# maelaubert/VulkanSift

Hardware: AMD Instinct MI355X
Metric: SIFT detect+match frames/sec (640x480, ~2k kp) (higher is better)
Workload: dtype f32

## Files before the change

vulkansift_amd/csrc/hip/features.hip:

```cpp
#include <hip/hip_runtime.h>
#include <stdint.h>
#include <stdlib.h>
#include <type_traits>

#include "../detmath.h"
#include "features_math.h"
#include "multi.h"
#include "records.h"
#include "vksift_hip.h"
#include "wave.h"

namespace
{

struct FeatArgs
{
  const float *gauss;
  uint32_t fp16;
  int w, h, pitch;
  uint64_t plane_stride, img_stride;
  uint8_t *feats;
  uint64_t feat_img_stride;
  uint32_t cap;
  uint32_t *found;
  uint32_t found_img_stride;
  float *ori_ang;
  uint32_t *ori_cnt;
  uint64_t ori_img_stride;
  uint32_t max_keep;
  uint32_t use_vlfeat;
  const float *desc_fp_tab;
  uint32_t desc_fp_tab_len;
  uint32_t sec;
};

struct ImageView
{
  uint32_t found, n;
  uint8_t *feats;
  int w, h, pitch;
  size_t plane;
};
__device__ __forceinline__ ImageView image_view(const FeatArgs &a, int b)
{
  ImageView v;
  v.found = a.found[(size_t)b * a.found_img_stride];
  v.n = v.found < a.cap ? v.found : a.cap;
  v.feats = a.feats + (size_t)b * a.feat_img_stride;
  v.w = a.w, v.h = a.h, v.pitch = a.pitch;
  v.plane = (size_t)a.plane_stride;
  return v;
}

struct KeyHead
{
  const float *rec;
  float scale_x, scale_y, sigma, theta;
  int octave_idx;
  __amdgpu_buffer_rsrc_t rs;
};
template <bool F16>
__device__ __forceinline__ KeyHead keypoint_head(const FeatArgs &a, const ImageView &v, int b, uint32_t k)
{
  KeyHead kh;
  kh.rec = (const float *)(v.feats + (size_t)k * VKSIFT_RECORD_BYTES);
  const uint32_t scale_idx = (uint32_t)__builtin_amdgcn_readfirstlane((int)((const uint32_t *)kh.rec)[4]);
  kh.octave_idx = ((const int *)kh.rec)[5];
  kh.sigma = kh.rec[6];
  kh.scale_x = kh.rec[2], kh.scale_y = kh.rec[3], kh.theta = kh.rec[7];
  kh.rs = layer_rsrc(a.gauss, (size_t)b * a.img_stride + (size_t)scale_idx * v.plane, v.pitch, v.h, F16);
  return kh;
}

template <bool IMG_FAST, bool F16>
__global__ void __launch_bounds__(256) k_orientation(Multi<FeatArgs> m)
{
  const VBlock vb = vblock(m);
  const FeatArgs &a = m.oct[vb.o];
  __shared__ uint32_t s_hist[4][36];
  const int lane = threadIdx.x & 63, wave = threadIdx.x >> 6;
  const int b = (int)(IMG_FAST ? vb.x : vb.y);
  const ImageView g = image_view(a, b);
  uint32_t *hist = s_hist[wave];

  const uint32_t bk = IMG_FAST ? vb.y : vb.x, nbk = IMG_FAST ? vb.gy : vb.gx;
  for (uint32_t k = bk * 4 + wave; k < g.n; k += nbk * 4)
  {
    if (lane < 36)
      hist[lane] = 0;
    __builtin_amdgcn_wave_barrier();
    float fp = 0.f;
    {
      const KeyHead kh = keypoint_head<F16>(a, g, b, k);
      float lambda = 1.5f * (kh.sigma * dm_pow2i(-kh.octave_idx));
      int r = (int)floorf(3 * lambda);
      float es = -1.f / (2.f * lambda * lambda);
      const bool may_clamp = (2.f * (float)(r + 1) * (float)(r + 1)) * es < -87.f;

      float gsum = 1.f;
      for (int cb = 0; cb <= r; cb += 64)
      {
        int i = cb + lane;
        float e = (i >= 1 && i <= r) ? dm_expf(es * (float)(i * i)) : 0.f;
        int lim = r - cb < 63 ? r - cb : 63;
        for (int j = 0; j <= lim; j++)
        {
          float ej = __shfl(e, j, 64);
          if (cb + j >= 1)
            gsum += 2.f * ej;
        }
      }
      float M = (gsum * gsum) * sqrtf(2.f);
      fp = (float)(1u << (uint32_t)(30 - dm_ceil_log2f(M)));

      float rsx = roundf(kh.scale_x), rsy = roundf(kh.scale_y);
      int box = 2 * r + 1;
      int npix = box * box;
      const float rbox = __builtin_amdgcn_rcpf((float)box);
      const bool small_box = box < 32768;
      const int step_q = small_box ? (int)(64.5f * rbox) : 64 / box, step_r = 64 - step_q * box;
      int py = small_box ? (int)(((float)lane + 0.5f) * rbox) : lane / box, px = lane - py * box;
      auto accumulate = [&](float sdx2, float tr, float tl, float td, float tu) {
        const float gradX = 0.5f * (tr - tl);
        const float gradY = 0.5f * (td - tu);
        const float xe = sdx2 * es;
        float e = dm_expf_core_nonpos(fmaxf(xe, -87.3f));
        if (may_clamp)
          e = xe < -87.3f ? 0.f : e;
        float ori, len;
        bool odd;
        grad_polar<true>(gradX, gradY, &ori, &len, &odd);
        float x36 = wrap_2pi(ori) * 36.f;
        float fbin = angle_bin<true>(x36);
        odd |= angle_bin_odd(x36);
        if (__builtin_expect(__ballot(odd) != 0ull, 0))
        {
          grad_polar<false>(gradX, gradY, &ori, &len, nullptr);
          fbin = angle_bin<false>(wrap_2pi(ori) * 36.f);
        }
        const float mag = e * len;
        int bin = (int)fbin;
        bin = bin >= 36 ? bin - 36 : bin;
        atomicAdd(&hist[bin], (uint32_t)(mag * fp));
      };
      const int cxi = (int)rsx, cyi = (int)rsy;
      const int pitch4 = g.pitch * 4;
      auto window = [&](auto INTERIOR) {
        for (int pix = lane; pix < npix; pix += 64)
        {
          const int dy = py - r, dx = px - r;
          px += step_r, py += step_q;
          if (px >= box)
            px -= box, py++;
          const float sdx = (rsx + (float)dx) - kh.scale_x;
          const float sdy = (rsy + (float)dy) - kh.scale_y;
          const float d2 = (sdx * sdx) + (sdy * sdy);
          if constexpr (decltype(INTERIOR)::value)
          {
            const unsigned v0 = (__umul24((unsigned)(cyi + dy - 1), (unsigned)g.pitch) + (unsigned)(cxi + dx - 1)) * 4u;
            accumulate(d2, tap_ld<F16>(kh.rs, v0 + 8u, pitch4), tap_ld<F16>(kh.rs, v0, pitch4), tap_ld<F16>(kh.rs, v0 + 4u, 2 * pitch4), tap_ld<F16>(kh.rs, v0 + 4u, 0));
          }
          else
          {
            const int gx = cxi + dx, gy = cyi + dy;
            if ((gx < 1 || gx >= (g.w - 1) || gy < 1 || gy >= (g.h - 1)) && (d2 > (float)(r * r)))
              continue;
            const bool xin = (unsigned)gx < (unsigned)g.w, yin = (unsigned)gy < (unsigned)g.h;
            const unsigned o0 = (__umul24((unsigned)gy, (unsigned)g.pitch) + (unsigned)gx) * 4u;
            const unsigned o_r = (yin && (unsigned)(gx + 1) < (unsigned)g.w) ? o0 + 4u : 0x80000000u;
            const unsigned o_l = (yin && (unsigned)(gx - 1) < (unsigned)g.w) ? o0 - 4u : 0x80000000u;
            const unsigned o_d = (xin && (unsigned)(gy + 1) < (unsigned)g.h) ? (__umul24((unsigned)(gy + 1), (unsigned)g.pitch) + (unsigned)gx) * 4u : 0x80000000u;
            const unsigned o_u = (xin && (unsigned)(gy - 1) < (unsigned)g.h) ? (__umul24((unsigned)(gy - 1), (unsigned)g.pitch) + (unsigned)gx) * 4u : 0x80000000u;
            accumulate(d2, tap_ld<F16>(kh.rs, o_r, 0), tap_ld<F16>(kh.rs, o_l, 0), tap_ld<F16>(kh.rs, o_d, 0), tap_ld<F16>(kh.rs, o_u, 0));
          }
        }
      };
      if (cxi - r >= 1 && cxi + r <= g.w - 2 && cyi - r >= 1 && cyi + r <= g.h - 2)
        window(std::true_type{});
      else
        window(std::false_type{});
    }
    __builtin_amdgcn_wave_barrier();
    {
      const int li = lane < 36 ? lane : 0;
      uint32_t hv = hist[li];
      const int lm = (li + 35) % 36, lp = (li + 1) % 36;
#pragma unroll
      for (int it = 0; it < 6; it++)
      {
        uint32_t hm = __shfl(hv, lm, 64), hp = __shfl(hv, lp, 64);
        hv = (uint32_t)dm_div_3((float)(hm + hv + hp));
      }
      uint32_t hm = __shfl(hv, lm, 64), hp = __shfl(hv, lp, 64);
      const uint32_t mx = wave_max_u32(lane < 36 ? hv : 0u);
      bool peak = lane < 36 && ((float)hv >= (0.8f * (float)mx)) && (hv > hm) && (hv > hp);
      unsigned long long pm = __ballot(peak);
      uint32_t npk = (uint32_t)__popcll(pm);
      if (peak)
      {
        uint32_t rank = ballot_rank(pm, lane);
        if (rank < a.max_keep)
        {
          uint32_t num = hm - hp;
          uint32_t den = hm - (2u * hv) + hp;
          float idx = (float)lane + 0.5f * ((float)num / (float)den);
          float ang = (idx + 0.5f) * (2.f * PI_F) / 36.f;
          a.ori_ang[((size_t)b * a.ori_img_stride + k) * VKSIFT_HIP_MAX_ORI + rank] = ang;
        }
      }
      if (lane == 0)
        a.ori_cnt[(size_t)b * a.ori_img_stride + k] = npk < a.max_keep ? npk : a.max_keep;
    }
    __builtin_amdgcn_wave_barrier();
  }
}

__global__ void __launch_bounds__(1024) k_orientation_finalize(Multi<FeatArgs> m)
{
  __shared__ uint32_t wave_tot[16];
  __shared__ uint32_t carry_s;
  const VBlock vb = vblock(m);
  const FeatArgs &a = m.oct[vb.o];
  const int b = (int)vb.x;
  const int lane = threadIdx.x & 63, wave = threadIdx.x >> 6;
  const ImageView g = image_view(a, b);
  const uint32_t *cnt = a.ori_cnt + (size_t)b * a.ori_img_stride;
  const float *ang = a.ori_ang + (size_t)b * a.ori_img_stride * VKSIFT_HIP_MAX_ORI;
  if (threadIdx.x == 0)
    carry_s = 0;
  __syncthreads();
  for (uint32_t base = 0; base < g.n; base += 1024)
  {
    uint32_t k = base + threadIdx.x;
    uint32_t c = k < g.n ? cnt[k] : 0u;
    uint32_t v = c > 1 ? c - 1 : 0u;
    const uint32_t incl = wave_scan_incl_u32(v, lane);
    if (lane == 63)
      wave_tot[wave] = incl;
    __syncthreads();
    uint32_t wave_base = 0;
    for (int wv = 0; wv < wave; wv++)
      wave_base += wave_tot[wv];
    uint32_t carry = carry_s;
    uint32_t excl = carry + wave_base + incl - v;
    if (k < g.n && c >= 1)
    {
      uint32_t *rec = (uint32_t *)(g.feats + (size_t)k * VKSIFT_RECORD_BYTES);
      rec[7] = __float_as_uint(ang[(size_t)k * VKSIFT_HIP_MAX_ORI]);
      for (uint32_t j = 1; j < c; j++)
      {
        uint32_t idx = g.found + excl + (j - 1);
        if (idx < a.cap)
        {
          uint32_t *dst = (uint32_t *)(g.feats + (size_t)idx * VKSIFT_RECORD_BYTES);
#pragma unroll
          for (int q = 0; q < (int)VKSIFT_RECORD_HEAD_WORDS; q++)
            dst[q] = rec[q];
          dst[7] = __float_as_uint(ang[(size_t)k * VKSIFT_HIP_MAX_ORI + j]);
        }
      }
    }
    __syncthreads();
    if (threadIdx.x == 1023)
      carry_s = carry + wave_base + incl;
    __syncthreads();
  }
  if (threadIdx.x == 0)
    a.found[(size_t)b * a.found_img_stride] = g.found + carry_s;
}

__device__ __forceinline__ int smod8(int v) { return v & 7; }

struct DescCtx
{
  __amdgpu_buffer_rsrc_t rs;
  int pitch, pitch4;
  float scale_x, scale_y, rsx, rsy, kcos, ksin, kori, fp, bin_scale;
  int dx0, dx1, dy0, dy1;
  float offx, offy, ia0, ia1;
};

struct DescSample
{
  float ox, oy, mag;
  float xb;
};

struct DescTaps
{
  float up, lf, rt, dn;
};

__device__ __forceinline__ unsigned desc_tap_base(const DescCtx &c, int cdx, int cdy)
{
  const int ix = (int)c.rsx + cdx, iy = (int)c.rsy + cdy;
  return (__umul24((unsigned)(iy - 1), (unsigned)c.pitch) + (unsigned)(ix - 1)) * 4u;
}

template <bool F16>
__device__ __forceinline__ DescTaps desc_taps(const DescCtx &c, unsigned v0)
{
  DescTaps t;
  t.up = tap_ld<F16>(c.rs, v0 + 4u, 0);
  t.lf = tap_ld<F16>(c.rs, v0, c.pitch4);
  t.rt = tap_ld<F16>(c.rs, v0 + 8u, c.pitch4);
  t.dn = tap_ld<F16>(c.rs, v0 + 4u, 2 * c.pitch4);
  return t;
}

typedef uint32_t u32x2_t __attribute__((ext_vector_type(2)));
typedef uint32_t u32x4_t __attribute__((ext_vector_type(4)));
__device__ __forceinline__ void desc_taps_pair(const DescCtx &c, unsigned v0, DescTaps &a, DescTaps &b)
{
  const u32x2_t up = __builtin_amdgcn_raw_buffer_load_b64(c.rs, v0 + 4u, 0, 0);
  const u32x4_t mid = __builtin_amdgcn_raw_buffer_load_b128(c.rs, v0, c.pitch4, 0);
  const u32x2_t dn = __builtin_amdgcn_raw_buffer_load_b64(c.rs, v0 + 4u, 2 * c.pitch4, 0);
  a.up = __uint_as_float(up.x), b.up = __uint_as_float(up.y);
  a.lf = __uint_as_float(mid.x), b.lf = __uint_as_float(mid.y);
  a.rt = __uint_as_float(mid.z), b.rt = __uint_as_float(mid.w);
  a.dn = __uint_as_float(dn.x), b.dn = __uint_as_float(dn.y);
}

template <bool INRANGE>
__device__ __forceinline__ DescSample desc_sample(const DescCtx &c, int cdx, int cdy, const DescTaps &t, bool *odd)
{
  const float es = -1.f / (2.f * 2 * 2);
  float sdx = (c.rsx + (float)cdx) - c.scale_x;
  float sdy = (c.rsy + (float)cdy) - c.scale_y;
  DescSample r;
  r.ox = c.kcos * sdx + c.ksin * sdy;
  r.oy = c.kcos * sdy - c.ksin * sdx;
  float gradX = 0.5f * (t.rt - t.lf);
  float gradY = 0.5f * (t.dn - t.up);
  float ori, root;
  grad_polar<INRANGE>(gradX, gradY, &ori, &root, odd);
  ori = wrap_2pi(ori);
  ori = wrap_2pi(ori - c.kori);
  r.mag = dm_expf_core_nonpos(es * ((r.ox * r.ox) + (r.oy * r.oy))) * root;
  r.xb = ori * c.bin_scale;
  return r;
}

constexpr int DESC_PAD = 1, DESC_ROW_CELLS = 8;
constexpr int DESC_HIST_WORDS = (4 + 2 * DESC_PAD) * DESC_ROW_CELLS * 16;
constexpr int DESC_WORK_WORDS = ((4 + DESC_PAD - 1) * DESC_ROW_CELLS + (4 + DESC_PAD - 1) + 1) * 16;
static_assert(DESC_WORK_WORDS <= DESC_HIST_WORDS && DESC_WORK_WORDS % 2 == 0, "64-bit slots");
__device__ __forceinline__ int desc_cell_word(int cell)
{
  return (((cell >> 2) + DESC_PAD) * DESC_ROW_CELLS + (cell & 3) + DESC_PAD) * 16;
}
__device__ __forceinline__ uint32_t desc_hist_read(const uint32_t *s_work, int t)
{
  const int cw = desc_cell_word(t >> 3), bin = t & 7;
  return s_work[cw + 2 * bin] + s_work[cw + 2 * ((bin + 7) & 7) + 1];
}

__device__ __forceinline__ void desc_scatter(const DescCtx &c, const DescSample &r, float fbin, bool live, uint32_t *s_work)
{
  float fhx = r.ox + 2.f, fhy = r.oy + 2.f;
  const float flx = floorf(fhx - 0.5f), fly = floorf(fhy - 0.5f), flb = floorf(fbin);
  int hx = (int)flx, hy = (int)fly, hb = (int)flb;
  float rhx = fhx - (flx + 0.5f), rhy = fhy - (fly + 0.5f), rb = fbin - flb;
  const float magfp = r.mag * c.fp;
  const unsigned b0 = (unsigned)smod8(hb);
  const unsigned pair = b0 * 8u;
  const bool okx[2] = {live && (unsigned)hx < 4u, live && (unsigned)(hx + 1) < 4u};
  const bool oky[2] = {(unsigned)hy < 4u, (unsigned)(hy + 1) < 4u};
  char *base = (char *)s_work + ((unsigned)((hy + DESC_PAD) * (DESC_ROW_CELLS * 64) + (hx + DESC_PAD) * 64) + pair);
#pragma unroll
  for (int i = 0; i < 2; i++)
#pragma unroll
    for (int j = 0; j < 2; j++)
    {
      const float w = fabsf(1.f - (float)i - rhx) * fabsf(1.f - (float)j - rhy);
      const uint32_t v0 = (uint32_t)((w * fabsf(1.f - 0.f - rb)) * magfp);
      const uint32_t v1 = (uint32_t)((w * fabsf(1.f - 1.f - rb)) * magfp);
      if (okx[i] && oky[j])
        atomicAdd((unsigned long long *)(base + (j * DESC_ROW_CELLS * 64 + i * 64)), ((unsigned long long)v1 << 32) | v0);
    }
}

constexpr int DESC_MAX_ROWS = 256;

template <bool CAN_POST>
__device__ __forceinline__ void desc_dense_prologue(const FeatArgs &a, const vksift_hip_DenseRows &dr, int b, bool first_block, int tid, uint32_t *s_row0)
{
  if (!(dr.desc || (CAN_POST && dr.post)))
    return;
  const uint32_t *fsec = a.found + (size_t)b * a.found_img_stride - a.sec;
  uint32_t row0 = 0, total = 0;
#pragma unroll
  for (uint32_t j = 0; j < 16u; j++)
    if (j < dr.nsec)
    {
      const uint32_t f = fsec[j], n = f < dr.sec_cap[j] ? f : dr.sec_cap[j];
      row0 += j < a.sec ? n : 0u;
      total += n;
    }
  if (tid == 0)
    *s_row0 = row0;
  if (a.sec == 0 && first_block)
  {
    if (CAN_POST && dr.post && (uint32_t)tid < dr.found_post_n)
      dr.found_post[(size_t)b * dr.found_post_n + tid] = fsec[tid];
    if (dr.desc && tid == 0)
      dr.n[(size_t)b * dr.n_img_stride] = total;
    if (dr.desc && total < 2u && tid < 64)
    {
      uint32_t *z = (uint32_t *)(dr.desc + (size_t)b * dr.desc_img_stride);
      if (tid >= (int)total * 32)
        z[tid] = 0u;
      if (tid < 2 && tid >= (int)total)
        dr.norm[(size_t)b * dr.norm_img_stride + tid] = 128u * 128u * 128u;
    }
  }
}

__device__ __forceinline__ int desc_radius(float sigma, int octave_idx, float *lambda)
{
  float scale_factor = dm_pow2i(octave_idx);
  *lambda = 3.0f * (sigma / scale_factor);
  float radius = sqrtf(2.f) * *lambda * 5.f * 0.5f;
  return (int)floorf(radius + 0.5f);
}

__device__ __forceinline__ DescCtx desc_setup(const FeatArgs &a, const ImageView &g, const KeyHead &kh)
{
  DescCtx c;
  c.scale_x = kh.scale_x, c.scale_y = kh.scale_y, c.kori = kh.theta;
  c.rs = kh.rs;
  c.pitch = g.pitch, c.pitch4 = g.pitch * 4;
  c.bin_scale = a.use_vlfeat ? 8.f : -8.f;
  float lambda;
  const int R = desc_radius(kh.sigma, kh.octave_idx, &lambda);
  float sn, cs;
  dm_sincosf(c.kori, &sn, &cs);
  c.kcos = cs / lambda, c.ksin = sn / lambda;
  uint32_t ti = (uint32_t)(R / 2);
  c.fp = a.desc_fp_tab[ti < a.desc_fp_tab_len ? ti : a.desc_fp_tab_len - 1];
  c.rsx = roundf(c.scale_x), c.rsy = roundf(c.scale_y);

  const int cxi = (int)c.rsx, cyi = (int)c.rsy;
  c.dx0 = max(-R, 1 - cxi), c.dx1 = min(R, g.w - 2 - cxi);
  c.dy0 = max(-R, 1 - cyi), c.dy1 = min(R, g.h - 2 - cyi);
  c.offx = c.rsx - c.scale_x, c.offy = c.rsy - c.scale_y;
  c.ia0 = __builtin_amdgcn_rcpf(c.kcos), c.ia1 = __builtin_amdgcn_rcpf(-c.ksin);
  return c;
}

struct DescRows
{
  int *lo;
  uint32_t *cnt;
  const uint32_t *pre;
  int y0, nrows;
};

template <int NT>
__device__ __forceinline__ void desc_row_spans(const DescCtx &c, const DescRows &rows, int tid)
{
  const float T = 2.5f + 0.01f;
  for (int row = tid; row < rows.nrows; row += NT)
  {
    const float fy = (float)(rows.y0 + row) + c.offy;
    float lo = (float)c.dx0 - 0.5f, hi = (float)c.dx1 + 0.5f;
#pragma unroll
    for (int e = 0; e < 2; e++)
    {
      const float aa = e == 0 ? c.kcos : -c.ksin, ia = e == 0 ? c.ia0 : c.ia1;
      const float bb = e == 0 ? c.ksin * fy : c.kcos * fy;
      if (fabsf(aa) > 1e-12f)
      {
        const float ctr = -bb * ia - c.offx, half = T * fabsf(ia);
        lo = fmaxf(lo, ctr - half);
        hi = fminf(hi, ctr + half);
      }
      else if (!(fabsf(bb) < T))
        hi = lo - 2.f;
    }
    const int ilo = (int)ceilf(lo - 0.01f), ihi = (int)floorf(hi + 0.01f);
    const int xl = max(ilo, c.dx0), xh = min(ihi, c.dx1);
    rows.lo[row] = xl;
    rows.cnt[row] = xh >= xl ? (uint32_t)(xh - xl + 1) : 0u;
  }
}

__device__ __forceinline__ void desc_row_prefix(const DescRows &rows, uint32_t *pre, int lane)
{
  uint32_t carry = 0;
  for (int base = 0; base < rows.nrows; base += 64)
  {
    const int i = base + lane;
    const uint32_t v = i < rows.nrows ? rows.cnt[i] : 0u;
    const uint32_t incl = wave_scan_incl_u32(v, lane);
    if (i < rows.nrows)
      pre[i] = carry + incl - v;
    carry += __shfl(incl, 63, 64);
  }
  if (lane == 0)
    pre[rows.nrows] = carry;
}

struct DescRun
{
  uint32_t steps;
  uint32_t sidx, send;
  int row, cdx;
  uint32_t row_end;
};
template <int NWV>
__device__ __forceinline__ DescRun desc_run(const DescRows &rows, int wave, int lane)
{
  const uint32_t *s_pre = rows.pre;
  const uint32_t N = s_pre[rows.nrows];
  const uint32_t T = (N + 63u) / 64u, tq = T / NWV, tr = T % NWV;
  DescRun r;
  r.steps = tq + ((uint32_t)wave < tr ? 1u : 0u);
  const uint32_t step0 = (uint32_t)wave * tq + min((uint32_t)wave, tr);
  r.sidx = min(N, step0 * 64u + (uint32_t)lane * r.steps);
  r.send = min(N, r.sidx + r.steps);
  int row = 0;
  if (r.sidx < r.send)
  {
    int lo_r = 0, hi_r = rows.nrows - 1;
    while (lo_r < hi_r)
    {
      const int mid = (lo_r + hi_r + 1) >> 1;
      if (s_pre[mid] <= r.sidx)
        lo_r = mid;
      else
        hi_r = mid - 1;
    }
    row = lo_r;
    while (s_pre[row + 1] <= r.sidx)
      row++;
  }
  r.row = row;
  r.cdx = rows.lo[row] + (int)(r.sidx - s_pre[row]);
  r.row_end = s_pre[row + 1];
  return r;
}

__device__ __forceinline__ bool desc_next_sample(const DescRows &rows, DescRun &r, int &sx, int &sy)
{
  const bool live = r.sidx < r.send;
  if (live && r.sidx >= r.row_end)
  {
    do
      r.row++;
    while (rows.pre[r.row + 1] <= r.sidx);
    r.row_end = rows.pre[r.row + 1];
    r.cdx = rows.lo[r.row];
  }
  sx = r.cdx, sy = rows.y0 + r.row;
  r.cdx++, r.sidx++;
  return live;
}

template <bool F16>
__device__ __forceinline__ void desc_step_pair(const DescCtx &c, const DescRows &rows, DescRun &run, uint32_t *s_work)
{
  int sx[2], sy[2];
  const bool live[2] = {desc_next_sample(rows, run, sx[0], sy[0]), desc_next_sample(rows, run, sx[1], sy[1])};
  DescTaps t0, t1;
  const unsigned v0 = desc_tap_base(c, sx[0], sy[0]);
  if (F16)
  {
    t0 = desc_taps<F16>(c, v0);
    t1 = desc_taps<F16>(c, desc_tap_base(c, sx[1], sy[1]));
  }
  else
  {
    desc_taps_pair(c, v0, t0, t1);
    if (live[1] && !(sy[1] == sy[0] && sx[1] == sx[0] + 1))
      t1 = desc_taps<F16>(c, desc_tap_base(c, sx[1], sy[1]));
  }
  bool o0, o1;
  DescSample s0 = desc_sample<true>(c, sx[0], sy[0], t0, &o0), s1 = desc_sample<true>(c, sx[1], sy[1], t1, &o1);
  float f0 = angle_bin<true>(s0.xb), f1 = angle_bin<true>(s1.xb);
  o0 |= angle_bin_odd(s0.xb), o1 |= angle_bin_odd(s1.xb);
  if (__builtin_expect(__ballot(o0 || o1) != 0ull, 0))
  {
    s0 = desc_sample<false>(c, sx[0], sy[0], t0, nullptr), s1 = desc_sample<false>(c, sx[1], sy[1], t1, nullptr);
    f0 = angle_bin<false>(s0.xb), f1 = angle_bin<false>(s1.xb);
  }
  desc_scatter(c, s0, f0, live[0], s_work);
  desc_scatter(c, s1, f1, live[1], s_work);
}

template <bool F16>
__device__ __forceinline__ void desc_step_odd(const DescCtx &c, const DescRows &rows, DescRun &run, uint32_t *s_work)
{
  int sx, sy;
  const bool live = desc_next_sample(rows, run, sx, sy);
  const DescSample s0 = desc_sample<false>(c, sx, sy, desc_taps<F16>(c, desc_tap_base(c, sx, sy)), nullptr);
  desc_scatter(c, s0, angle_bin<false>(s0.xb), live, s_work);
}

__device__ __forceinline__ uint32_t desc_byte(float v) { return (v != v) ? 0u : (v < 0.f ? 0u : (v > 255.f ? 255u : (uint32_t)v)); }
__device__ __forceinline__ void desc_bytes(const uint32_t *s_work, int ln, uint32_t &b0, uint32_t &b1)
{
  uint32_t w0 = desc_hist_read(s_work, ln), w1 = desc_hist_read(s_work, ln + 64);
  float norm = sqrtf((float)wave_sum_u32(w0 * w0 + w1 * w1));
  uint32_t lim = (uint32_t)(norm * 0.2f);
  w0 = w0 < lim ? w0 : lim;
  w1 = w1 < lim ? w1 : lim;
  norm = sqrtf((float)wave_sum_u32(w0 * w0 + w1 * w1));
  float scale = 512.f / norm;
  b0 = desc_byte((float)w0 * scale), b1 = desc_byte((float)w1 * scale);
}
__device__ __forceinline__ uint32_t desc_pack4(uint32_t byte, int ln)
{
  uint32_t p = byte << ((uint32_t)(ln & 3) * 8u);
  p |= __shfl_xor(p, 1, 64);
  p |= __shfl_xor(p, 2, 64);
  return p;
}
__device__ __forceinline__ void desc_store_dwords(uint32_t *dst, int ln, uint32_t p0, uint32_t p1)
{
  if ((ln & 3) == 0)
  {
    dst[ln >> 2] = p0;
    dst[16 + (ln >> 2)] = p1;
  }
}
__device__ __forceinline__ void desc_post_record(const vksift_hip_DenseRows &dr, int b, uint32_t row, const float *rec, int ln, uint32_t p0, uint32_t p1)
{
  const uint32_t j = (uint32_t)ln & 15u;
  const uint32_t d0 = __shfl(p0, (int)(4u * j), 64), d1 = __shfl(p1, (int)(4u * j), 64);
  uint32_t *out = (uint32_t *)(dr.post + (size_t)b * dr.post_img_stride) + (size_t)row * VKSIFT_RECORD_WORDS;
  if (ln < 32)
    out[(int)VKSIFT_RECORD_HEAD_WORDS + ln] = ln < 16 ? d0 : d1;
  else if (ln < (int)VKSIFT_RECORD_WORDS)
    out[ln - 32] = ((const uint32_t *)rec)[ln - 32];
}
__device__ __forceinline__ void desc_dense_row(const vksift_hip_DenseRows &dr, int b, uint32_t row0, uint32_t k, int ln, uint32_t p0, uint32_t p1)
{
  uint32_t *dense = (uint32_t *)(dr.desc + (size_t)b * dr.desc_img_stride) + (size_t)row0 * 32;
  uint32_t *dense_norm = dr.norm + (size_t)b * dr.norm_img_stride + row0;
  uint32_t s2 = __builtin_amdgcn_udot4(p0, p0, 0u, false), s1 = __builtin_amdgcn_udot4(p0, 0x01010101u, 0u, false);
  s2 = __builtin_amdgcn_udot4(p1, p1, s2, false), s1 = __builtin_amdgcn_udot4(p1, 0x01010101u, s1, false);
#pragma unroll
  for (int dlt = 32; dlt >= 4; dlt >>= 1)
  {
    s2 += __shfl_xor(s2, dlt, 64);
    s1 += __shfl_xor(s1, dlt, 64);
  }
  desc_store_dwords(dense + (size_t)k * 32, ln, p0, p1);
  if (ln == 0)
    dense_norm[k] = s2 - 256u * s1 + 128u * 128u * 128u;
}

template <bool CAN_POST>
__device__ __forceinline__ void desc_epilogue(const vksift_hip_DenseRows &dr, const ImageView &g, int b, uint32_t k, const float *rec, const uint32_t *s_work,
                                              const uint32_t *s_row0, int lane)
{
  int ln = lane;
  asm volatile("" : "+v"(ln));
  uint32_t b0, b1;
  desc_bytes(s_work, ln, b0, b1);
  const uint32_t p0 = desc_pack4(b0, ln), p1 = desc_pack4(b1, ln);
  desc_store_dwords((uint32_t *)(g.feats + (size_t)k * VKSIFT_RECORD_BYTES + VKSIFT_RECORD_DESC_AT), ln, p0, p1);
  if (CAN_POST && dr.post)
    desc_post_record(dr, b, *s_row0 + k, rec, ln, p0, p1);
  if (dr.desc)
    desc_dense_row(dr, b, *s_row0, k, ln, p0, p1);
}

template <int NW>
__device__ __forceinline__ void desc_sync()
{
  if (NW == 1)
    __builtin_amdgcn_wave_barrier();
  else
    __syncthreads();
}
template <int NW, int NPH, int MAXR, bool PAIRS, bool CAN_POST, bool F16>
__device__ __forceinline__ void desc_keypoint(const FeatArgs &a, const vksift_hip_DenseRows &dr, const ImageView &g, int b, uint32_t k, int wave, int tid,
                                              uint32_t *s_work, int *s_lo, uint32_t *s_cnt, uint32_t *s_pre, const uint32_t *s_row0)
{
  desc_sync<NW>();
  {
    int zt = tid;
    if (PAIRS)
      asm volatile("" : "+v"(zt));
    for (int i = zt; i < 256; i += 64 * NW)
      s_work[desc_cell_word(i >> 4) + (i & 15)] = 0;
  }

  const KeyHead kh = keypoint_head<F16>(a, g, b, k);
  const DescCtx c = desc_setup(a, g, kh);
  const int bh = c.dy1 - c.dy0 + 1;
  for (int rb = 0; rb < bh; rb += MAXR)
  {
    const DescRows rows{s_lo, s_cnt, s_pre, c.dy0 + rb, min(MAXR, bh - rb)};
    int rt = tid;
    if (PAIRS)
      asm volatile("" : "+v"(rt));
    desc_sync<NW>();
    desc_row_spans<64 * NW>(c, rows, rt);
    desc_sync<NW>();
    desc_row_prefix(rows, s_pre, rt & 63);
    __builtin_amdgcn_wave_barrier();
#pragma unroll 1
    for (int ph = 0; ph < NPH; ph++)
    {
      int pt = tid;
      if (PAIRS)
        asm volatile("" : "+v"(pt));
      DescRun run = desc_run<NW * NPH>(rows, wave * NPH + ph, pt & 63);
      uint32_t it = 0;
      for (; it + 1 < run.steps; it += 2)
        desc_step_pair<F16>(c, rows, run, s_work);
      if (it < run.steps)
        desc_step_odd<F16>(c, rows, run, s_work);
    }
  }
  desc_sync<NW>();
  if (wave == 0)
    desc_epilogue<CAN_POST>(dr, g, b, k, kh.rec, s_work, s_row0, tid & 63);
}

#ifndef DESC_SOLO_PHASES
#define DESC_SOLO_PHASES 4
#endif
constexpr int DESC_SOLO_MAX_R = 63;
__device__ __forceinline__ bool desc_pair_small(const ImageView &g, uint32_t k0, int lane, uint32_t solo_r)
{
  const float *rec = (const float *)(g.feats + (size_t)(k0 + ((uint32_t)lane & 1u)) * VKSIFT_RECORD_BYTES);
  float lambda;
  const int R = desc_radius(rec[6], ((const int *)rec)[5], &lambda);
  return __ballot(R > (int)solo_r) == 0ull;
}

template <int NWV, bool IMG_FAST, bool F16>
__global__ void __launch_bounds__(64 * NWV) __attribute__((amdgpu_waves_per_eu((NWV == 2 && !F16) ? 8 : 6, 8)))
k_descriptor(Multi<FeatArgs> m, vksift_hip_DenseRows dr, uint32_t solo_r)
{
  const VBlock vb = vblock(m);
  const FeatArgs &a = m.oct[vb.o];
  constexpr int NSOLO = NWV == 2 ? 2 : 1;
  static_assert(2 * DESC_SOLO_MAX_R + 1 <= DESC_MAX_ROWS / 2, "a solo window's rows fit half of the row arrays");
  __shared__ __attribute__((aligned(8))) uint32_t s_work[NSOLO][DESC_WORK_WORDS];
  __shared__ int s_row_lo[DESC_MAX_ROWS];
  __shared__ uint32_t s_row_cnt[DESC_MAX_ROWS];
  __shared__ uint32_t s_row_pre[NWV][DESC_MAX_ROWS + 1];
  __shared__ uint32_t s_row0;
  const int tid = threadIdx.x, lane = threadIdx.x & 63, wave = __builtin_amdgcn_readfirstlane(threadIdx.x >> 6);
  const int b = (int)(IMG_FAST ? vb.x : vb.y);
  const ImageView g = image_view(a, b);
  const uint32_t bk = IMG_FAST ? vb.y : vb.x, nbk = IMG_FAST ? vb.gy : vb.gx;
  constexpr bool CAN_POST = NWV == 4;
  desc_dense_prologue<CAN_POST>(a, dr, b, bk == 0, tid, &s_row0);

  const uint32_t per = (NWV == 2 && solo_r != 0u) ? 2u : 1u;
  if (per == 2u)
    __syncthreads();
  for (uint32_t k0 = bk * per; k0 < g.n; k0 += nbk * per)
  {
    if constexpr (NWV == 2)
      if (per == 2u && k0 + 1u < g.n && desc_pair_small(g, k0, lane, solo_r))
      {
        constexpr int HALF = DESC_MAX_ROWS / 2;
        desc_keypoint<1, DESC_SOLO_PHASES, HALF, true, CAN_POST, F16>(a, dr, g, b, k0 + (uint32_t)wave, 0, lane, s_work[wave], s_row_lo + wave * HALF, s_row_cnt + wave * HALF,
                                              s_row_pre[wave], &s_row0);
        continue;
      }
    const uint32_t k1 = min(k0 + per, g.n);
    for (uint32_t k = k0; k < k1; k++)
      desc_keypoint<NWV, 1, DESC_MAX_ROWS, NWV == 2, CAN_POST, F16>(a, dr, g, b, k, wave, tid, s_work[0], s_row_lo, s_row_cnt, s_row_pre[wave], &s_row0);
  }
}

FeatArgs make_args(const vksift_hip_OctaveJob *job)
{
  FeatArgs a;
  a.gauss = job->gauss;
  a.fp16 = job->fp16;
  a.w = (int)job->w, a.h = (int)job->h, a.pitch = (int)job->pitch;
  a.plane_stride = job->plane_stride, a.img_stride = job->img_stride;
  a.feats = job->feats, a.feat_img_stride = job->feat_img_stride, a.cap = job->cap;
  a.found = job->found, a.found_img_stride = job->found_img_stride;
  a.ori_ang = job->ori_ang, a.ori_cnt = job->ori_cnt, a.ori_img_stride = job->ori_img_stride;
  uint32_t mk = job->max_ori == 0 ? VKSIFT_HIP_MAX_ORI : job->max_ori;
  a.max_keep = mk > VKSIFT_HIP_MAX_ORI ? VKSIFT_HIP_MAX_ORI : mk;
  a.use_vlfeat = job->use_vlfeat;
  a.desc_fp_tab = job->desc_fp_tab, a.desc_fp_tab_len = job->desc_fp_tab_len;
  a.sec = job->sec_index;
  return a;
}

bool img_fast(uint32_t batch, bool descriptor)
{
  return batch > 1 && !descriptor;
}

bool add_octave(Multi<FeatArgs> &m, const FeatArgs &a, bool img_fast, uint32_t batch, uint32_t blocks)
{
  return multi_add(m, a, img_fast ? batch : blocks, img_fast ? blocks : batch, 1u);
}

uint32_t expected_keypoints(const vksift_hip_OctaveJob *job, uint32_t batch)
{
  const uint32_t pixels_per_keypoint = 512;
  if (batch < 8u)
    return 0xFFFFFFFFu;
  const uint64_t n = (uint64_t)job->w * job->h / pixels_per_keypoint;
  return n < 32u ? 32u : (n > 0xFFFFFFFFull ? 0xFFFFFFFFu : (uint32_t)n);
}

uint32_t octave_blocks(const vksift_hip_OctaveJob *job, uint32_t batch, uint32_t kp_per_block, uint32_t cap_blocks)
{
  const uint32_t dense = expected_keypoints(job, batch);
  uint32_t blocks = ((job->cap < dense ? job->cap : dense) + (kp_per_block - 1)) / kp_per_block;
  if (blocks > cap_blocks)
    blocks = cap_blocks;
  return blocks == 0 ? 1 : blocks;
}

}

static int orientation_run(const vksift_hip_OctaveJob *jobs, uint32_t n, uint32_t batch, hipStream_t hs)
{
  Multi<FeatArgs> mo, mf;
  mo.n = mf.n = 0;
  const bool f = img_fast(batch, false);
  uint32_t cap_blocks = 16384u / batch;
  cap_blocks = cap_blocks < 32u ? 32u : (cap_blocks > 1024u ? 1024u : cap_blocks);
  for (uint32_t i = 0; i < n; i++)
  {
    const FeatArgs a = make_args(&jobs[i]);
    if (!add_octave(mo, a, f, batch, octave_blocks(&jobs[i], batch, 4, cap_blocks)) || !multi_add(mf, a, batch, 1u, 1u))
      return (int)hipErrorInvalidValue;
  }
  const bool f16 = mo.oct[0].fp16 != 0;
  const dim3 grid(mo.start[mo.n]);
  with_bool(f, [&](auto IMG_FAST) {
    with_bool(f16, [&](auto F16) { hipLaunchKernelGGL((k_orientation<decltype(IMG_FAST)::value, decltype(F16)::value>), grid, dim3(256), 0, hs, mo); });
  });
  hipLaunchKernelGGL(k_orientation_finalize, dim3(mf.start[mf.n]), dim3(1024), 0, hs, mf);
  return (int)hipGetLastError();
}

static int descriptor_run(const vksift_hip_OctaveJob *jobs, uint32_t n, uint32_t batch, const vksift_hip_DenseRows &dr, hipStream_t hs)
{
  Multi<FeatArgs> md;
  md.n = 0;
  const bool f = img_fast(batch, true);
  const bool two_waves = batch >= 8u;
  const int tune_r = vksift_hip_tune_get(VKSIFT_TUNE_DESC_SOLO_R);
  const uint32_t solo_r = !two_waves || tune_r <= 0 ? 0u : (tune_r > DESC_SOLO_MAX_R ? (uint32_t)DESC_SOLO_MAX_R : (uint32_t)tune_r);
  for (uint32_t i = 0; i < n; i++)
    if (!add_octave(md, make_args(&jobs[i]), f, batch, octave_blocks(&jobs[i], batch, solo_r ? 2 : 1, 2048)))
      return (int)hipErrorInvalidValue;
  if (dr.post && two_waves)
    return (int)hipErrorInvalidValue;
  const bool f16 = md.oct[0].fp16 != 0;
  const dim3 grid(md.start[md.n]);
  with_bool(two_waves, [&](auto TWO) {
    constexpr int NWV = decltype(TWO)::value ? 2 : 4;
    with_bool(f, [&](auto IMG_FAST) {
      with_bool(f16, [&](auto F16) {
        hipLaunchKernelGGL((k_descriptor<NWV, decltype(IMG_FAST)::value, decltype(F16)::value>), grid, dim3(64 * NWV), 0, hs, md, dr, solo_r);
      });
    });
  });
  return (int)hipGetLastError();
}

template <typename F>
static int for_runs(const vksift_hip_OctaveJob *jobs, uint32_t n_jobs, F run)
{
  for (uint32_t i0 = 0; i0 < n_jobs;)
  {
    uint32_t i1 = i0 + 1;
    while (i1 < n_jobs && i1 - i0 < multi_run_max() && jobs[i1].fp16 == jobs[i0].fp16)
      i1++;
    const int e = run(jobs + i0, i1 - i0);
    if (e)
      return e;
    i0 = i1;
  }
  return 0;
}

extern "C"
{
  int vksift_hip_orientations_multi(const vksift_hip_OctaveJob *jobs, uint32_t n_jobs, uint32_t batch, vksift_hip_stream s)
  {
    if (batch == 0)
      return 0;
    return for_runs(jobs, n_jobs, [&](const vksift_hip_OctaveJob *j, uint32_t n) { return orientation_run(j, n, batch, (hipStream_t)s); });
  }

  int vksift_hip_descriptors_multi_dense(const vksift_hip_OctaveJob *jobs, uint32_t n_jobs, uint32_t batch, const vksift_hip_DenseRows *dense,
                                         vksift_hip_stream s)
  {
    if (batch == 0)
      return 0;
    vksift_hip_DenseRows dr = {};
    if (dense)
    {
      const bool rows = dense->desc != NULL, post = dense->post != NULL;
      if ((!rows && !post) || (rows && (!dense->norm || !dense->n)) || (post && (!dense->found_post || dense->found_post_n > 64u)) || dense->nsec == 0 ||
          dense->nsec > 16u)
        return (int)hipErrorInvalidValue;
      for (uint32_t i = 0; i < n_jobs; i++)
        if (jobs[i].sec_index >= dense->nsec)
          return (int)hipErrorInvalidValue;
      dr = *dense;
    }
    return for_runs(jobs, n_jobs, [&](const vksift_hip_OctaveJob *j, uint32_t n) { return descriptor_run(j, n, batch, dr, (hipStream_t)s); });
  }

  int vksift_hip_descriptors_multi(const vksift_hip_OctaveJob *jobs, uint32_t n_jobs, uint32_t batch, vksift_hip_stream s)
  {
    return vksift_hip_descriptors_multi_dense(jobs, n_jobs, batch, nullptr, s);
  }

  int vksift_hip_orientations(const vksift_hip_OctaveJob *job, uint32_t batch, vksift_hip_stream s) { return vksift_hip_orientations_multi(job, 1, batch, s); }

  int vksift_hip_descriptors(const vksift_hip_OctaveJob *job, uint32_t batch, vksift_hip_stream s) { return vksift_hip_descriptors_multi(job, 1, batch, s); }
}
```

Measured before the change: 26680.

## Partition descriptor samples into same-row horizontal pairs instead of individual samples

The descriptor work split now counts row-aligned pairs of adjacent pixels (ceil(cnt/2) per row) instead of single samples. Each lane step handles two horizontally adjacent samples, so the paired tap load always applies and the fallback reload and odd-tail step go away. Row advance uses the span end x instead of prefix lookups. The cost is wasted lanes when a row has odd length, since the second sample is masked, and some imbalance from the coarser work units.

```diff
diff --git a/vulkansift_amd/csrc/hip/features.hip b/vulkansift_amd/csrc/hip/features.hip
--- a/vulkansift_amd/csrc/hip/features.hip
+++ b/vulkansift_amd/csrc/hip/features.hip
@@ -491,7 +491,7 @@
   for (int base = 0; base < rows.nrows; base += 64)
   {
     const int i = base + lane;
-    const uint32_t v = i < rows.nrows ? rows.cnt[i] : 0u;
+    const uint32_t v = i < rows.nrows ? (rows.cnt[i] + 1u) >> 1 : 0u;
     const uint32_t incl = wave_scan_incl_u32(v, lane);
     if (i < rows.nrows)
       pre[i] = carry + incl - v;
@@ -506,19 +506,19 @@
   uint32_t steps;
   uint32_t sidx, send;
   int row, cdx;
-  uint32_t row_end;
+  int xend;
 };
 template <int NWV>
 __device__ __forceinline__ DescRun desc_run(const DescRows &rows, int wave, int lane)
 {
   const uint32_t *s_pre = rows.pre;
-  const uint32_t N = s_pre[rows.nrows];
-  const uint32_t T = (N + 63u) / 64u, tq = T / NWV, tr = T % NWV;
+  const uint32_t P = s_pre[rows.nrows];
+  const uint32_t T = (P + 63u) / 64u, tq = T / NWV, tr = T % NWV;
   DescRun r;
   r.steps = tq + ((uint32_t)wave < tr ? 1u : 0u);
   const uint32_t step0 = (uint32_t)wave * tq + min((uint32_t)wave, tr);
-  r.sidx = min(N, step0 * 64u + (uint32_t)lane * r.steps);
-  r.send = min(N, r.sidx + r.steps);
+  r.sidx = min(P, step0 * 64u + (uint32_t)lane * r.steps);
+  r.send = min(P, r.sidx + r.steps);
   int row = 0;
   if (r.sidx < r.send)
   {
@@ -536,65 +536,55 @@
       row++;
   }
   r.row = row;
-  r.cdx = rows.lo[row] + (int)(r.sidx - s_pre[row]);
-  r.row_end = s_pre[row + 1];
+  const int lo = rows.lo[row];
+  r.cdx = lo + 2 * (int)(r.sidx - s_pre[row]);
+  r.xend = lo + (int)rows.cnt[row];
   return r;
 }
 
-__device__ __forceinline__ bool desc_next_sample(const DescRows &rows, DescRun &r, int &sx, int &sy)
-{
-  const bool live = r.sidx < r.send;
-  if (live && r.sidx >= r.row_end)
-  {
+__device__ __forceinline__ void desc_next_slot(const DescRows &rows, DescRun &r, int &sx, int &sy, bool live[2])
+{
+  live[0] = r.sidx < r.send;
+  if (live[0] && r.cdx >= r.xend)
+  {
+    uint32_t n;
     do
-      r.row++;
-    while (rows.pre[r.row + 1] <= r.sidx);
-    r.row_end = rows.pre[r.row + 1];
+      n = rows.cnt[++r.row];
+    while (n == 0u);
     r.cdx = rows.lo[r.row];
+    r.xend = r.cdx + (int)n;
   }
   sx = r.cdx, sy = rows.y0 + r.row;
-  r.cdx++, r.sidx++;
-  return live;
+  live[1] = live[0] && r.cdx + 1 < r.xend;
+  r.cdx += 2, r.sidx++;
 }
 
 template <bool F16>
 __device__ __forceinline__ void desc_step_pair(const DescCtx &c, const DescRows &rows, DescRun &run, uint32_t *s_work)
 {
-  int sx[2], sy[2];
-  const bool live[2] = {desc_next_sample(rows, run, sx[0], sy[0]), desc_next_sample(rows, run, sx[1], sy[1])};
+  int sx, sy;
+  bool live[2];
+  desc_next_slot(rows, run, sx, sy, live);
   DescTaps t0, t1;
-  const unsigned v0 = desc_tap_base(c, sx[0], sy[0]);
+  const unsigned v0 = desc_tap_base(c, sx, sy);
   if (F16)
   {
     t0 = desc_taps<F16>(c, v0);
-    t1 = desc_taps<F16>(c, desc_tap_base(c, sx[1], sy[1]));
+    t1 = desc_taps<F16>(c, desc_tap_base(c, sx + 1, sy));
   }
   else
-  {
     desc_taps_pair(c, v0, t0, t1);
-    if (live[1] && !(sy[1] == sy[0] && sx[1] == sx[0] + 1))
-      t1 = desc_taps<F16>(c, desc_tap_base(c, sx[1], sy[1]));
-  }
   bool o0, o1;
-  DescSample s0 = desc_sample<true>(c, sx[0], sy[0], t0, &o0), s1 = desc_sample<true>(c, sx[1], sy[1], t1, &o1);
+  DescSample s0 = desc_sample<true>(c, sx, sy, t0, &o0), s1 = desc_sample<true>(c, sx + 1, sy, t1, &o1);
   float f0 = angle_bin<true>(s0.xb), f1 = angle_bin<true>(s1.xb);
   o0 |= angle_bin_odd(s0.xb), o1 |= angle_bin_odd(s1.xb);
   if (__builtin_expect(__ballot(o0 || o1) != 0ull, 0))
   {
-    s0 = desc_sample<false>(c, sx[0], sy[0], t0, nullptr), s1 = desc_sample<false>(c, sx[1], sy[1], t1, nullptr);
+    s0 = desc_sample<false>(c, sx, sy, t0, nullptr), s1 = desc_sample<false>(c, sx + 1, sy, t1, nullptr);
     f0 = angle_bin<false>(s0.xb), f1 = angle_bin<false>(s1.xb);
   }
   desc_scatter(c, s0, f0, live[0], s_work);
   desc_scatter(c, s1, f1, live[1], s_work);
-}
-
-template <bool F16>
-__device__ __forceinline__ void desc_step_odd(const DescCtx &c, const DescRows &rows, DescRun &run, uint32_t *s_work)
-{
-  int sx, sy;
-  const bool live = desc_next_sample(rows, run, sx, sy);
-  const DescSample s0 = desc_sample<false>(c, sx, sy, desc_taps<F16>(c, desc_tap_base(c, sx, sy)), nullptr);
-  desc_scatter(c, s0, angle_bin<false>(s0.xb), live, s_work);
 }
 
 __device__ __forceinline__ uint32_t desc_byte(float v) { return (v != v) ? 0u : (v < 0.f ? 0u : (v > 255.f ? 255u : (uint32_t)v)); }
@@ -709,11 +699,8 @@
       if (PAIRS)
         asm volatile("" : "+v"(pt));
       DescRun run = desc_run<NW * NPH>(rows, wave * NPH + ph, pt & 63);
-      uint32_t it = 0;
-      for (; it + 1 < run.steps; it += 2)
+      for (uint32_t it = 0; it < run.steps; it++)
         desc_step_pair<F16>(c, rows, run, s_work);
-      if (it < run.steps)
-        desc_step_odd<F16>(c, rows, run, s_work);
     }
   }
   desc_sync<NW>();
```

Measured after the change: 27120 (median of 6 runs). 1.02x the previous value.
